# wenet-e2e/wesep

Hardware: AMD Instinct MI355X
Metric: utterances/sec (4 s, 16 kHz, 2-spk) fwd+bwd, pBSRNN (higher is better)
Workload: dtype bf16x3+fp16x2+fp16x1 split products (+fp8 lo terms), fp32 accumulate; 1 GPU; pBSRNN FiLM multi-fuse, 6 repeats, feature_dim 128, fixed 256-d embeddings; fwd + SI-SDR + bwd + per-tensor clip + Adam-L2; bf16x3 (x-projections, projections, d(hcat), BN / mask GEMMs) + fp16x2 (recurrent products of all four recurrence kernels, d(xn)) + fp16x1 (LSTM weight gradients); 2-byte saved gates / d(gates); fp32 accumulate; BPTT kernels: W_hh as fp16 hi + block-scaled FP8 lo; the lo term; rows_per_gpu=32, global_rows=32, samples_per_row=64000, parallelism=dp1

## Files before the change

### include/wesep_hip.h

```cpp
#ifndef WESEP_HIP_H_
#define WESEP_HIP_H_

#ifdef __cplusplus
extern "C" {
#endif

#define WS_ABI_VERSION 20
#define WS_OK 0
#define WS_ERR_INVALID (-1)
#define WS_ERR_LAUNCH (-2)

int ws_abi_version(void);
const char* ws_last_error(void);

#define WS_PROF_LSTM_FWD 0
#define WS_PROF_LSTM_BWD 1
#define WS_PROF_GEMM_NT 2
#define WS_PROF_GEMM_TN 3
#define WS_PROF_NKINDS 4
int ws_prof_enable(int on);
int ws_prof_collect(int kind, double* total_ms, long long* launches);
int ws_debug_dirty_lds(float value, int nblocks, int spins, float* sink, void* stream);
int ws_debug_occupy(int nblocks, int usec, const unsigned* stop, float* sink, void* stream);

// ... 592 lines not shown

#define WS_RESAMPLE_MAX_UD 1024
#define WS_RESAMPLE_MAX_K 4096
int ws_resample_geom(int rate_in, int rate_out, int* U, int* D, int* w, int* K);
int ws_resample_taps(int rate_in, int rate_out, float* taps);
int ws_resample_fwd(const float* x, long long ldx, int R, int n_in, int rate_in, int rate_out, const float* taps, float* y,
                    long long ldy, void* stream);
int ws_resample_stream_fwd(const float* buf, long long ldb, int R, int rate_in, int rate_out, const float* taps, int lead,
                           int n_valid, int final, int g_first, int n_out, float* y, long long ldy, int hist_from, int hist_len,
                           float* hist, long long ldh, void* stream);

typedef struct ws_resample_row {
  long long in_off, taps_off, out_off, hist_off;
  int U, D, K;
  int lead, n_valid, final, g_first, n_out, hist_from, hist_len;
} ws_resample_row;
typedef struct ws_rows_copy_row {
  long long src_off, dst_off;
  int len, fill;
} ws_rows_copy_row;
typedef struct ws_window_resample_row {
  long long in_off, taps_off, out_off;
  int U, D, K;
  int lead, n_valid, final, g_first, p_first, L, fill;
} ws_window_resample_row;
int ws_resample_stream_rows_fwd(const ws_resample_row* rows, const ws_resample_row* d_rows, int A, const float* buf,
                                long long n_buf, const float* taps, long long n_taps, float* y, long long n_y, float* hist,
                                long long n_hist, void* stream);
int ws_rows_copy_fwd(const ws_rows_copy_row* rows, const ws_rows_copy_row* d_rows, int A, const float* src, long long n_src,
                     float* dst, long long n_dst, void* stream);
int ws_window_resample_rows_fwd(const ws_window_resample_row* rows, const ws_window_resample_row* d_rows, int A, const float* buf,
                                long long n_buf, const float* taps, long long n_taps, float* y, long long n_y, void* stream);

#ifdef __cplusplus
}
#endif
#endif
```

### wesep_amd/_lib.py

```python
import ctypes as C
import os

import numpy as np
import torch

_HERE = os.path.dirname(os.path.abspath(__file__))
LIB_PATH = os.environ.get("WESEP_HIP_LIB") or os.path.join(_HERE, "libwesep_hip.so")

WS_OK = 0
PROF_LSTM_FWD, PROF_LSTM_BWD, PROF_GEMM_NT, PROF_GEMM_TN = 0, 1, 2, 3
LSTM_H = 256
ABI_VERSION = 20
GATES_F32, GATES_H2, GATES_H2S, GATES_H2F = 0, 1, 2, 3
DGATES_EXP = 8


def dgates_scale(amax_bits: int) -> float:
    e = (int(amax_bits) >> 23) & 0xFF
    return 1.0 if e in (0, 255) else 2.0 ** (min(max(DGATES_EXP + 254 - e, 1), 253) - 127)


LSTM_F32_MT1, LSTM_F32_MT2, LSTM_BF16X3, LSTM_BF16X3_BLK, LSTM_BF16X3_BLK16 = 1, 2, 3, 4, 5
LSTM_FWD_H2P = 16
LSTM_C16 = 32
# ... 53 lines not shown
    _fields_ = [(n, _p) for n in ("G", "X", "slab", "bslab")] + \
               [(n, _ll) for n in ("ldg", "slab_stride", "bslab_stride")] + \
               [(n, _i) for n in ("M", "Nn", "nsplit", "tiles_per_split")] + [("conv", ConvView)]


class GroupsGeom(C.Structure):
    _fields_ = [("band_w", _p), ("band_off", _p), ("gs1", _ll), ("gs2", _ll), ("rs", _ll),
                ("ngroups", _i), ("gdiv", _i), ("L", _i), ("W", _i), ("nbands", _i), ("pad_", _i)]


class LstmArgs(C.Structure):
    _fields_ = [(n, _p) for n in ("gates", "cbuf", "hcat", "dhcat", "wpack")] + \
               [(n, _ll) for n in ("sq_s1", "sq_s2", "step_rows")] + \
               [(n, _i) for n in ("nseq", "sq_div", "L", "mode")] + [("run_if", _p)] + \
               [("gates_in", _p), ("dgates", _p), ("gfmt", _i), ("rfmt", _i), ("amax", _p)] + \
               [("dxn", _p), ("dxn_dir_stride", _ll), ("wxpack", _p)]


class SeqMapC(C.Structure):
    _fields_ = [("sq_s1", _ll), ("sq_s2", _ll), ("step_rows", _ll), ("nseq", _i), ("sq_div", _i), ("L", _i), ("nvalid", _i)]


class GemmP2BArgs(C.Structure):
    _fields_ = [(n, _p) for n in ("A", "Wpack", "bias", "C", "A_bl", "stats", "gamma", "beta")] + \
               [("sm", SeqMapC)] + [(n, _ll) for n in ("lda", "st_m1", "st_m2", "st_base")] + \
               [(n, _i) for n in ("st_div1", "st_div2", "N", "K")] + [("run_if", _p), ("amax", _p), ("A_bl16", _p)]


class GemmB2PArgs(C.Structure):
    _fields_ = [(n, _p) for n in ("A", "Wpack", "bias", "R", "C")] + [("sm", SeqMapC), ("ldc", _ll), ("N", _i), ("K", _i),
                                                                         ("a_fmt", _i), ("pad_", _i), ("amax", _p), ("a16_out", _p)]


class FilmDesc(C.Structure):
    _fields_ = [("a", _p), ("b", _p), ("a0", _f), ("rows_per_r", _i)]


class GemmTNBArgs(C.Structure):
    _fields_ = [(n, _p) for n in ("G", "A0", "A1", "slab", "bslab", "aslab")] + \
               [(n, _ll) for n in ("slab_stride", "bslab_stride", "aslab_stride")] + \
               [(n, _i) for n in ("g_width", "g_off", "g_cols", "a0_width", "a0_off", "a0_cols", "a0_shift",
                                  "a1_width", "a1_off", "a1_cols", "a1_shift", "nblk", "L", "nsplit",
                                  "blocks_per_split", "g_fmt")] + [("amax", _p), ("a_fmt", _i), ("pad_", _i)]


class LstmClusterArgs(C.Structure):
    _fields_ = [(n, _p) for n in ("gates", "cbuf", "hcat", "dhcat", "whh_f", "whh_r", "xchg", "flags", "status")] + \
               [("nseq", _i), ("L", _i), ("dbg", _i), ("gfmt", _i), ("gates_in", _p)]


class LstmCluster2Args(C.Structure):
    _fields_ = [(n, _p) for n in ("gates", "cbuf", "hcat", "xn", "wcat", "bcat", "whh_f", "whh_r", "xchg", "tword", "status")] + \
               [("nseq", _i), ("L", _i), ("dbg", _i), ("rfmt", _i), ("dbg_buf", _p)]


class LstmPairArgs(C.Structure):
    _fields_ = [(n, _p) for n in ("gates", "cbuf", "dhcat", "wpack", "xchg", "flags", "status", "dbg_buf")] + \
               [("nseq", _i), ("L", _i), ("dbg", _i), ("gfmt", _i), ("dgates", _p), ("amax", _p), ("rfmt", _i), ("pad_", _i)]


class Bands(C.Structure):
    _fields_ = [("band_of_bin", _p), ("band_f0", _p), ("band_bw", _p), ("nband", _i), ("nbins", _i)]


GROUP_NT_DTYPE = np.dtype([("W", "<u8"), ("bias", "<u8"), ("gamma", "<u8"), ("beta", "<u8"),
                           ("a_off", "<i8"), ("c_off", "<i8"), ("st_base", "<i8"),
                           ("K", "<i4"), ("N", "<i4"), ("ldw", "<i4"), ("pad_", "<i4")])
GROUP_TN_DTYPE = np.dtype([("gamma", "<u8"), ("beta", "<u8"), ("g_off", "<i8"), ("a_off", "<i8"),
                           ("st_base", "<i8"), ("out_off", "<i8"), ("bout_off", "<i8"),
                           ("Nn", "<i4"), ("Kk", "<i4"), ("pad0_", "<i4"), ("pad1_", "<i4")])
TENSOR_REF_DTYPE = np.dtype([("param", "<u8"), ("grad", "<u8"), ("exp_avg", "<u8"),
                             ("exp_avg_sq", "<u8"), ("numel", "<i8")])
assert GROUP_NT_DTYPE.itemsize == 72 and GROUP_TN_DTYPE.itemsize == 72 and TENSOR_REF_DTYPE.itemsize == 40

class LstmFusedArgs(C.Structure):
    _fields_ = [("gates", _p), ("cbuf", _p), ("hcat", _p), ("xn", _p), ("wpack", _p), ("bias", _p),
                ("nseq", _i), ("L", _i), ("gfmt", _i), ("hfmt", _i)]


LSTM_FUSED_PACK_FLOATS = 2 * 8 * 24 * 4 * 2 * 64 * 4
LSTM_DX_PACK_FLOATS = 16 * (48 * 1024 + 64) // 4

_SIGS = {
    "ws_abi_version": (_i, []),
    "ws_last_error": (C.c_char_p, []),
    "ws_prof_enable": (_i, [_i]),
    "ws_prof_collect": (_i, [_i, C.POINTER(C.c_double), C.POINTER(_ll)]),
    "ws_debug_dirty_lds": (_i, [_f, _i, _i, _p, _p]),
    "ws_debug_occupy": (_i, [_i, _i, _p, _p, _p]),
    "ws_pack_w_f16": (_i, [_p, _i, _i, _ll, _i, _i, _p, _p]),
    "ws_pack_w_f16f8": (_i, [_p, _i, _i, _ll, _i, _p, _p]),
    "ws_gemm_nt": (_i, [C.POINTER(GemmNTArgs), _p]),
    "ws_gemm_tn": (_i, [C.POINTER(GemmTNArgs), _p]),
    "ws_reduce_slabs": (_i, [_p, _i, _ll, _ll, _p, _i, _ll, _p]),
    "ws_transpose": (_i, [_p, _i, _i, _ll, _p, _p]),
    "ws_group_stats": (_i, [_p, C.POINTER(GroupsGeom), _f, _p, _p]),
    "ws_group_stats_len": (_i, [_p, C.POINTER(GroupsGeom), _p, _i, _f, _p, _p]),
    "ws_gn_bwd_reduce": (_i, [_p, _p, _p, _p, _p, C.POINTER(GroupsGeom), _p, _p]),
    "ws_gn_bwd_apply": (_i, [_p, _p, _p, _p, _p, _p, _p, C.POINTER(GroupsGeom), _p, _p]),
    "ws_gn_param_grad": (_i, [_p, _p, _p, C.POINTER(GroupsGeom), _i, _p, _p]),
    "ws_gn_bwd_fused": (_i, [_p, _p, _p, _p, _p, C.POINTER(GroupsGeom), _i, _p, _p, _p, _p, _p]),
    "ws_gn_bwd_fused2": (_i, [_p, _p, _p, _p, _p, _p, C.POINTER(GroupsGeom), _i, _p, _p, _p, _p, _p]),
    "ws_gn_bwd_apply_pg": (_i, [_p, _p, _p, _p, _p, _p, C.POINTER(GroupsGeom), _p, _p, _p, _p, _p]),
    "ws_group_stats_film": (_i, [_p, C.POINTER(FilmDesc), C.POINTER(GroupsGeom), _f, _p, _p]),
    "ws_gn_bwd_reduce_film": (_i, [_p, C.POINTER(FilmDesc), _p, _p, _p, C.POINTER(GroupsGeom), _p, _p]),
    "ws_gn_bwd_apply_pg_film": (_i, [_p, C.POINTER(FilmDesc), _p, _p, _p, _p, _p, C.POINTER(GroupsGeom), _p, _p, _p, _p,
                                     _p, _p, _p, _p, _p]),
    "ws_lstm_pack": (_i, [_p, _p, _p, _p, _i, _p]),
    "ws_lstm_fwd": (_i, [C.POINTER(LstmArgs), _p]),
    "ws_lstm_bwd": (_i, [C.POINTER(LstmArgs), _p]),
    "ws_lstm_fwd_cluster": (_i, [C.POINTER(LstmClusterArgs), _p]),
    "ws_lstm_bwd_cluster": (_i, [C.POINTER(LstmClusterArgs), _p]),
    "ws_lstm_fwd_cluster2": (_i, [C.POINTER(LstmCluster2Args), _p]),
    "ws_lstm_pack_pair": (_i, [_p, _p, _p, _p]),
    "ws_lstm_pack_pair_f16": (_i, [_p, _p, _p, _p]),
    "ws_lstm_pack_pair_f8": (_i, [_p, _p, _p, _p]),
    "ws_lstm_pack_pair_f8mx": (_i, [_p, _p, _p, _p]),
    "ws_lstm_pack_bwd_f8": (_i, [_p, _p, _p, _p]),
    "ws_lstm_pack_dx_f8": (_i, [_p, _p, _p]),
    "ws_lstm_bwd_pair": (_i, [C.POINTER(LstmPairArgs), _p]),
    "ws_lstm_cat_ih": (_i, [_p, _p, _p, _p, _p, _p, _i, _p, _p, _p]),
    "ws_pack_w": (_i, [_p, _i, _i, _ll, _i, _i, _p, _p]),
    "ws_gemm_p2b": (_i, [C.POINTER(GemmP2BArgs), _p]),
    "ws_gemm_p2b_len": (_i, [C.POINTER(GemmP2BArgs), _p, _i, _p]),
    "ws_gemm_b2p": (_i, [C.POINTER(GemmB2PArgs), _p]),
    "ws_gemm_p2b_film": (_i, [C.POINTER(GemmP2BArgs), C.POINTER(FilmDesc), _p]),
    "ws_gemm_b2p_film": (_i, [C.POINTER(GemmB2PArgs), C.POINTER(FilmDesc), _p]),
    "ws_gemm_tnb": (_i, [C.POINTER(GemmTNBArgs), _p]),
    "ws_gemm_tnb_h16": (_i, [C.POINTER(GemmTNBArgs), _p]),
    "ws_stft_bandsplit": (_i, [_p, _i, _i, C.POINTER(Bands), _p, _p]),
    "ws_stft_bandsplit_len": (_i, [_p, _i, _i, _p, C.POINTER(Bands), _p, _p]),
    "ws_mask_istft_frames": (_i, [_p, _p, _i, _i, C.POINTER(Bands), _p, _p]),
    "ws_istft_ola": (_i, [_p, _i, _i, _i, _p, _p]),
    "ws_istft_ola_len": (_i, [_p, _i, _i, _i, _p, _p, _p]),
    "ws_mask_istft_bwd": (_i, [_p, _p, _p, _i, _i, _i, C.POINTER(Bands), _p, _p]),
    "ws_affine_fwd": (_i, [_p, _p, _p, _f, _ll, _i, _i, _p, _p]),
    "ws_affine_bwd": (_i, [_p, _p, _p, _f, _ll, _i, _i, _i, _p, _p, _p, _p, _p, _p, _p]),
    "ws_sisdr_fwd": (_i, [_p, _p, _i, _i, _f, _p, _p, _p]),
    "ws_sisdr_bwd": (_i, [_p, _p, _p, _p, _i, _i, _p, _p]),
    "ws_flat_stats": (_i, [_p, _i, _ll, C.c_float, _i, _p, _p, _p]),
    "ws_prelu_fwd": (_i, [_p, _p, _p, _ll, _i, _i, _p, _p]),
    "ws_prelu_bwd": (_i, [_p, _p, _p, _ll, _p, _p, _i, _p]),
    "ws_dwconv_fwd": (_i, [_p, _p, _p, _p, _p, _p, _i, _i, _i, _i, _i, _i, _p, _p]),
    "ws_dwconv_bwd": (_i, [_p, _p, _p, _p, _p, _p, _i, _i, _i, _i, _i, _i, _p, _i, _i, _p, _p]),
    "ws_dwconv_ex_fwd": (_i, [_p, _p, _p, _p, _p, _p, _i, _i, _i, _i, _i, _i, _i, _p, _p]),
    "ws_dwconv_ex_bwd": (_i, [_p, _p, _p, _p, _p, _p, _i, _i, _i, _i, _i, _i, _i, _p, _i, _i, _p, _p]),
    "ws_chan_sums": (_i, [_p, _p, _p, _i, _i, _i, _i, _i, _p, _p]),
    "ws_norm_ab": (_i, [_p, _p, _i, _i, _ll, _p, _p]),
    "ws_norm_bwd_apply_cl": (_i, [_p, _p, _p, _p, _p, _p, _ll, _i, _i, _p, _p]),
    "ws_maskmul_fwd": (_i, [_p, _ll, _p, _ll, _i, _p, _p]),
    "ws_maskmul_bwd": (_i, [_p, _p, _ll, _p, _ll, _i, _p, _ll, _p, _p]),
    "ws_relu_mask": (_i, [_p, _p, _ll, _p]),
    "ws_ola_fwd": (_i, [_p, _p, _i, _i, _i, _i, _i, _p, _p]),
    "ws_ola_bwd": (_i, [_p, _i, _i, _i, _i, _i, _p, _p]),
    "ws_sum_partial": (_i, [_p, _ll, _p, _i, _p]),
    "ws_bn_stats": (_i, [_p, _ll, _i, C.c_float, C.c_float, _p, _p, _i, _p, _p, _p]),
    "ws_bn_prelu_fwd": (_i, [_p, _p, _p, _p, _p, _p, _ll, _i, _p, _p, _p]),
    "ws_bn_bwd": (_i, [_p, _p, _p, _p, _ll, _i, _i, _p, _p, _p, _p]),
    "ws_maxpool3_fwd": (_i, [_p, _i, _i, _i, _p, _p]),
    "ws_maxpool3_bwd": (_i, [_p, _p, _i, _i, _i, _p, _p]),
# ... 155 lines not shown
```

### wesep_amd/dev.py

```python
import ctypes as C
import os
from typing import NamedTuple, Optional

import numpy as np
import torch

from . import _lib as L

BIG = 1 << 30


def gemm_mode() -> str:
    return os.environ.get("WESEP_GEMM", "bf16x3")


def _mode_bit(mode):
    return 4 if (mode or gemm_mode()) == "bf16x3" else 0
GN_EPS = float(np.finfo(np.float32).eps)


class Rows(NamedTuple):
    div: int
    s1: int
    s2: int
# ... 58 lines not shown
    ldp: int = 0


def _set_conv(a, conv: Optional[ConvView]):
    if conv is not None:
        a.conv.on = 1
        (a.conv.mode, a.conv.H, a.conv.W, a.conv.C, a.conv.Ho, a.conv.Wo, a.conv.k, a.conv.sh, a.conv.sw,
         a.conv.p, a.conv.dil, a.conv.ldp) = conv


def gemm_nt(*, A, a_rows: Rows, M: int, C_out, c_rows: Rows, N=0, K=0, W=None, ldw=0, bias=None,
            R=None, T=None, stats=None, gamma=None, beta=None, stat_map: Optional[StatMap] = None,
            act=0, groups=None, ngroups=0, max_n=0, vec=3, a_off=0, c_off=0, w_off=0, mode=None,
            conv: Optional[ConvView] = None):
    for n, t in (("A", A), ("W", W), ("bias", bias), ("C", C_out), ("R", R), ("T", T),
                 ("stats", stats), ("gamma", gamma), ("beta", beta)):
        _chk(t, n)
    a = L.GemmNTArgs()
    a.A, a.W, a.bias, a.C = _p(A, a_off), _p(W, w_off), _p(bias), _p(C_out, c_off)
    a.R, a.T = _p(R, c_off), _p(T, c_off)
    a.stats, a.gamma, a.beta = _p(stats), _p(gamma), _p(beta)
    a.groups = C.c_void_p(groups.data_ptr()) if groups is not None else None
    a.a_div, a.a_s1, a.a_s2 = a_rows
    a.c_div, a.c_s1, a.c_s2 = c_rows
    sm = stat_map or StatMap(1, 0, 1, 0, 0)
    a.st_div1, a.st_m1, a.st_div2, a.st_m2, a.st_base = sm
    a.M, a.N, a.K, a.ldw = M, N, K, ldw
    a.act, a.ngroups, a.max_n, a.vec = act, ngroups, max_n, vec | _mode_bit(mode)
    _set_conv(a, conv)
    if ALG is not None and groups is None:
        a_elems = (M // (conv.Ho * conv.Wo)) * conv.H * conv.W * conv.C if conv is not None else M * K
        _alg("gemm_nt", 4 * (a_elems + M * N * (1 + (R is not None) + (T is not None)) + N * K), 2 * M * N * K)
    L.check(L.lib().ws_gemm_nt(C.byref(a), L.stream_ptr()), "ws_gemm_nt")


def tn_splits(M: int):
    nsplit = max(1, min(64, M // 2048))
    rows = -(-M // nsplit)
    rows = -(-rows // 32) * 32
    nsplit = -(-M // rows)
    return nsplit, rows


def gemm_tn(*, G, g_rows: Rows, A, a_rows: Rows, M: int, slab, slab_stride: int, nsplit: int,
            rows_per_split: int, Nn=0, Kk=0, bslab=None, bslab_stride=0, out_off=0, bout_off=0,
            stats=None, gamma=None, beta=None, stat_map: Optional[StatMap] = None,
            shift_rows=0, seq_div=1, seq_len=1, groups=None, ngroups=0, max_n=0, max_k=0, vec=1,
            g_off=0, a_off=0, mode=None, conv: Optional[ConvView] = None):
    for n, t in (("G", G), ("A", A), ("slab", slab), ("bslab", bslab), ("stats", stats),
                 ("gamma", gamma), ("beta", beta)):
        _chk(t, n)
    a = L.GemmTNArgs()
    a.G, a.A, a.slab, a.bslab = _p(G, g_off), _p(A, a_off), _p(slab), _p(bslab)
    a.stats, a.gamma, a.beta = _p(stats), _p(gamma), _p(beta)
    a.groups = C.c_void_p(groups.data_ptr()) if groups is not None else None
    a.g_div, a.g_s1, a.g_s2 = g_rows
    a.a_div, a.a_s1, a.a_s2 = a_rows
    sm = stat_map or StatMap(1, 0, 1, 0, 0)
    a.st_div1, a.st_m1, a.st_div2, a.st_m2, a.st_base = sm
    a.slab_stride, a.bslab_stride, a.out_off, a.bout_off = slab_stride, bslab_stride, out_off, bout_off
    a.M, a.Nn, a.Kk, a.rows_per_split, a.nsplit = M, Nn, Kk, rows_per_split, nsplit
    a.shift_rows, a.seq_div, a.seq_len = shift_rows, seq_div, seq_len
    a.ngroups, a.max_n, a.max_k, a.vec = ngroups, max_n, max_k, vec | _mode_bit(mode)
    _set_conv(a, conv)
    if ALG is not None and groups is None:
        a_elems = (M // (conv.Ho * conv.Wo)) * conv.H * conv.W * conv.C if conv is not None else M * Kk
# ... 2045 lines not shown
```

### wesep_amd/functional.py

```python
import os

import numpy as np
import torch

from . import _lib as L
from . import dev
from .dev import BIG, Geom, Rows, SeqMap, StatMap, flat
from .blstm_core import (G4, H, PAIR_STAMPS, PackCache, WeightPacks, WGradBox, WGradCarrierFn, _NO_CACHE,
                         _PROBE_SAT, _cluster_dbg, _empty, _h2_probe, _pair_dbg, _pending, _probe_round, _reduce_new,
                         _side_stream, amax_word, band_dx, band_rfmt, blstm_bptt, blstm_dxn, blstm_forward,
                         blstm_weight_grads, consume_once, defer_wgrad, dxn_fmt, flush_deferred_wgrads, keep_for_side,
                         make_plan, mark_wgrads_ready, pair_rfmt, tnb_a16, weight_grads, wgrad_hold, zero_words)

NBIN = 257
HOP = 128


def _need_cuda(t, who):
    if not t.is_cuda:
        raise L.WesepHipError(f"{who}: wesep_amd has no CPU path; move the model and inputs to the GPU")


def _view_maps(view, R, K, Tf, N):
    if view == "time":
# ... 440 lines not shown

    @staticmethod
    def backward(ctx, dout):
        z, e, W = ctx.saved_tensors
        dout = dout.contiguous()
        R, K, Tf, N = z.shape
        E = e.shape[1]
        P = R * K * Tf
        d = z.device
        ns = _affine_splits(K * Tf)
        dc_slab = _empty(d, ns, R, N)
        dev.affine_bwd(dout, None, None, 1.0, P, K * Tf, N, ns, None, None, dc_slab)
        dc = _reduce_new(dc_slab, ns, R * N, (R, N))
        dW = _empty(d, N, N + E)
        nsplit, rps = dev.tn_splits(P)
        slab = _empty(d, nsplit, N * N)
        dev.gemm_tn(G=dout, g_rows=flat(N), A=z, a_rows=flat(N), M=P, Nn=N, Kk=N, slab=slab,
                    slab_stride=N * N, nsplit=nsplit, rows_per_split=rps)
        dev.reduce_slabs(slab, nsplit, N * N, N * N, dW, w=N, ldo=N + E)
        dWe, db = _lin_bwd_w(dc, e)
        dev.reduce_slabs(dWe, 1, N * E, N * E, dW, w=E, ldo=N + E, out_off=N)
        dz = _empty(d, R, K, Tf, N)
        WxT = _empty(d, N, N)
        dev.transpose(W, N, N, N + E, WxT)
        dev.gemm_nt(A=dout, a_rows=flat(N), M=P, N=N, K=N, W=WxT, ldw=N, C_out=dz, c_rows=flat(N))
        de = _lin_bwd_x(dc, W, src_off=N, rows=N, cols=E, lds=N + E) if ctx.needs_input_grad[1] else None
        return dz, de, dW, db


def mask_nn() -> bool:
    return dev.gemm_mode() == "bf16x3" and os.environ.get("WESEP_GEMM_NN", "1") != "0"


class BandPlan:

    def __init__(self, band_width, feature_dim, device):
        self.dev = device
        self.bands = dev.BandTables(band_width, device)
        self.bw = [int(b) for b in band_width]
        self.f0 = [int(f) for f in self.bands.f0_host]
        self.K = len(self.bw)
        self.N = feature_dim
        N = feature_dim
        H1 = 4 * N
        self.bn_woff = np.concatenate([[0], np.cumsum([N * 2 * b for b in self.bw])]).astype(np.int64)
        self.m_w3off = np.concatenate([[0], np.cumsum([4 * b * H1 for b in self.bw])]).astype(np.int64)
        self.m_b3off = np.concatenate([[0], np.cumsum([4 * b for b in self.bw])]).astype(np.int64)
        self.bn_wT = _empty(device, int(self.bn_woff[-1]))
        self.m_w1T = _empty(device, self.K * N * H1)
        self.m_w2T = _empty(device, self.K * H1 * H1)
        self.m_w3T = _empty(device, int(self.m_w3off[-1]))
        self._cache = {}

    def _up(self, arr):
        return L.upload_struct_array(arr, self.dev)

    def _key(self, params, R, Tf):
        return (R, Tf) + tuple(p.data_ptr() for p in params)

    def bn_desc(self, params, R, Tf):
        key = ("bn",) + self._key(params, R, Tf)
        if key not in self._cache:
            K, N = self.K, self.N
            nt = np.zeros(K, dtype=L.GROUP_NT_DTYPE)
            tn = np.zeros(K, dtype=L.GROUP_TN_DTYPE)
            dx = np.zeros(K, dtype=L.GROUP_NT_DTYPE)
            for g in range(K):
                gw, gb, cw, cb = params[4 * g:4 * g + 4]
                bw2 = 2 * self.bw[g]
                nt[g] = (cw.data_ptr(), cb.data_ptr(), gw.data_ptr(), gb.data_ptr(),
                         2 * self.f0[g], g * Tf * N, g, bw2, N, bw2, 0)
                tn[g] = (gw.data_ptr(), gb.data_ptr(), g * Tf * N, 2 * self.f0[g], g,
                         int(self.bn_woff[g]), g * N, N, bw2, 0, 0)
                dx[g] = (self.bn_wT.data_ptr() + 4 * int(self.bn_woff[g]), 0, 0, 0,
                         g * Tf * N, 2 * self.f0[g], 0, N, bw2, N, 0)
            self._cache = {k: v for k, v in self._cache.items() if k[0] != "bn"}
            self._cache[key] = (self._up(nt), self._up(tn), self._up(dx))
        return self._cache[key]

    def mask_desc(self, params, R, Tf):
        nn = mask_nn()
        key = ("mask", nn) + self._key(params, R, Tf)
        if key not in self._cache:
            K, N = self.K, self.N
            H1 = 4 * N
            M = R * Tf
            d = {n: np.zeros(K, dtype=L.GROUP_NT_DTYPE) for n in ("l1", "l2", "l3", "dh2", "dh1", "dxn")}
            t = {n: np.zeros(K, dtype=L.GROUP_TN_DTYPE) for n in ("w3", "w2", "w1")}
            gtab = np.zeros(K, dtype=np.uint64)
            for g in range(K):
                gw, gb, w1, b1, w2, b2, w3, b3 = params[8 * g:8 * g + 8]
                bw4 = 4 * self.bw[g]
                hoff = g * M * H1
                zoff = g * Tf * N
                gtab[g] = gw.data_ptr()
                d["l1"][g] = (w1.data_ptr(), b1.data_ptr(), gw.data_ptr(), gb.data_ptr(), zoff, hoff, g, N, H1, N, 0)
                d["l2"][g] = (w2.data_ptr(), b2.data_ptr(), 0, 0, hoff, hoff, 0, H1, H1, H1, 0)
                d["l3"][g] = (w3.data_ptr(), b3.data_ptr(), 0, 0, hoff, 4 * self.f0[g], 0, H1, bw4, H1, 0)
                if nn:
                    d["dh2"][g] = (w3.data_ptr(), 0, 0, 0, 4 * self.f0[g], hoff, 0, bw4, H1, H1, 0)
                    d["dh1"][g] = (w2.data_ptr(), 0, 0, 0, hoff, hoff, 0, H1, H1, H1, 0)
                    d["dxn"][g] = (w1.data_ptr(), 0, 0, 0, hoff, zoff, 0, H1, N, N, 0)
                else:
                    d["dh2"][g] = (self.m_w3T.data_ptr() + 4 * int(self.m_w3off[g]), 0, 0, 0,
                                   4 * self.f0[g], hoff, 0, bw4, H1, bw4, 0)
                    d["dh1"][g] = (self.m_w2T.data_ptr() + 4 * g * H1 * H1, 0, 0, 0, hoff, hoff, 0, H1, H1, H1, 0)
                    d["dxn"][g] = (self.m_w1T.data_ptr() + 4 * g * N * H1, 0, 0, 0, hoff, zoff, 0, H1, N, H1, 0)
                t["w3"][g] = (0, 0, 4 * self.f0[g], hoff, 0, int(self.m_w3off[g]), int(self.m_b3off[g]), bw4, H1, 0, 0)
                t["w2"][g] = (0, 0, hoff, hoff, 0, g * H1 * H1, g * H1, H1, H1, 0, 0)
                t["w1"][g] = (gw.data_ptr(), gb.data_ptr(), hoff, zoff, g, g * H1 * N, g * H1, H1, N, 0, 0)
            self._cache = {k: v for k, v in self._cache.items() if k[0] != "mask"}
            out = {k: self._up(v) for k, v in d.items()}
            out.update({"t" + k: self._up(v) for k, v in t.items()})
            out["gamma_tab"] = torch.from_numpy(gtab.view(np.int64)).to(self.dev)
            self._cache[key] = out
        return self._cache[key]


def _band_split_fwd(wav, plan, params, lengths=None, frames=None):
    R, T = wav.shape
    K, N = plan.K, plan.N
    Tf = 1 + T // HOP
    M = R * Tf
    d = wav.device
    xbs = _empty(d, M, 2 * NBIN)
    geo = Geom(R * K, K, Tf * 2 * NBIN, 0, 2 * NBIN, Tf, 128, K, plan.bands.bw2, plan.bands.off2)
    stats = _empty(d, R * K, 2)
    if lengths is None:
        dev.stft_bandsplit(wav, plan.bands, xbs)
        dev.group_stats(xbs, geo, stats)
    else:
        dev.stft_bandsplit(wav, plan.bands, xbs, lengths=lengths)
        dev.group_stats(xbs, geo, stats, glen=frames, glen_div=K)
    nt, _, _ = plan.bn_desc(params, R, Tf)
    z0 = _empty(d, R, K, Tf, N)
    dev.gemm_nt(A=xbs, a_rows=flat(2 * NBIN), M=M, C_out=z0, c_rows=Rows(Tf, K * Tf * N, N),
                stats=stats, stat_map=StatMap(Tf, K, 1, 0, 0), groups=nt, ngroups=K, max_n=N, vec=0)
    return z0, xbs, stats


def _mask_decode_fwd(z, xbs, plan, T, params, lengths=None, frames=None):
    R, K, Tf, N = z.shape
    H1 = 4 * N
    M = R * Tf
    d = z.device
    D = plan.mask_desc(params, R, Tf)
    geo = Geom(R * K, 1, Tf * N, 0, N, Tf, N, K)
    stats = _empty(d, R * K, 2)
    if lengths is None:
        dev.group_stats(z, geo, stats)
    else:
        dev.group_stats(z, geo, stats, glen=frames, glen_div=K)
    h1, h2 = _empty(d, K, M, H1), _empty(d, K, M, H1)
    dev.gemm_nt(A=z, a_rows=Rows(Tf, K * Tf * N, N), M=M, C_out=h1, c_rows=flat(H1), stats=stats,
                stat_map=StatMap(Tf, K, 1, 0, 0), act=1, groups=D["l1"], ngroups=K, max_n=H1)
    dev.gemm_nt(A=h1, a_rows=flat(H1), M=M, C_out=h2, c_rows=flat(H1), act=1, groups=D["l2"],
                ngroups=K, max_n=H1)
    m3 = _empty(d, M, 4 * NBIN)
    dev.gemm_nt(A=h2, a_rows=flat(H1), M=M, C_out=m3, c_rows=flat(4 * NBIN), groups=D["l3"],
                ngroups=K, max_n=4 * max(plan.bw))
    fr = _empty(d, M, 512)
    dev.mask_istft_frames(xbs, m3, R, Tf, plan.bands, fr)
    est = _empty(d, R, T)
    if lengths is None:
        dev.istft_ola(fr, R, Tf, T, est)
    else:
        dev.istft_ola(fr, R, Tf, T, est, lengths=lengths)
    return est, stats, h1, h2, m3


def band_split_ragged(wav, plan, params, lengths, frames):
    _need_cuda(wav, "BSRNN")
    return _band_split_fwd(wav.contiguous(), plan, [p.detach() for p in params], lengths, frames)[:2]


def mask_decode_ragged(z, xbs, plan, T, params, lengths, frames):
    _need_cuda(z, "BSRNN")
    return _mask_decode_fwd(z.contiguous(), xbs, plan, T, [p.detach() for p in params], lengths, frames)[0]


class BandSplitFn(torch.autograd.Function):

    @staticmethod
    def forward(ctx, wav, plan, *params):
        _need_cuda(wav, "BSRNN")
        wav = wav.contiguous()
        R, T = wav.shape
        Tf = 1 + T // HOP
        z0, xbs, stats = _band_split_fwd(wav, plan, params)
        ctx.save_for_backward(xbs, stats, *params)
# ... 17 lines not shown
        nsplit, rps = dev.tn_splits(M)
        wtot = int(plan.bn_woff[-1])
        slab, bslab = _empty(d, nsplit, wtot), _empty(d, nsplit, K * N)
        dev.gemm_tn(G=dz0, g_rows=Rows(Tf, K * Tf * N, N), A=xbs, a_rows=flat(2 * NBIN), M=M, slab=slab,
                    slab_stride=wtot, bslab=bslab, bslab_stride=K * N, nsplit=nsplit, rows_per_split=rps,
                    stats=stats, stat_map=smap, groups=tn, ngroups=K, max_n=N, max_k=128, vec=0)
        dW = _reduce_new(slab, nsplit, wtot, (wtot,))
        dB = _reduce_new(bslab, nsplit, K * N, (K * N,))
        for g in range(K):
            bw2 = 2 * plan.bw[g]
            dev.transpose(params[4 * g + 2].reshape(N, bw2), N, bw2, bw2, plan.bn_wT,
                          dst_off=int(plan.bn_woff[g]))
        dxn = _empty(d, M, 2 * NBIN)
        dev.gemm_nt(A=dz0, a_rows=Rows(Tf, K * Tf * N, N), M=M, C_out=dxn, c_rows=flat(2 * NBIN),
                    groups=dxd, ngroups=K, max_n=128, vec=3)
        ns2 = min(64, R)
        pslab = _empty(d, ns2, K, 2, 128)
        dev.gn_param_grad(xbs, dxn, stats, geo, ns2, pslab)
        dgb = _reduce_new(pslab, ns2, K * 2 * 128, (K, 2, 128))
        grads = []
        for g in range(K):
            bw2 = 2 * plan.bw[g]
            o = int(plan.bn_woff[g])
            grads += [dgb[g, 0, :bw2], dgb[g, 1, :bw2], dW[o:o + N * bw2].view(N, bw2, 1), dB[g * N:(g + 1) * N]]
        return (None, None) + tuple(grads)


class MaskDecodeFn(torch.autograd.Function):

    @staticmethod
    def forward(ctx, z, xbs, plan, T, *params):
        _need_cuda(z, "BSRNN")
        z = z.contiguous()
        est, stats, h1, h2, m3 = _mask_decode_fwd(z, xbs, plan, T, params)
        ctx.save_for_backward(z, xbs, stats, h1, h2, m3, *params)
        ctx.plan, ctx.T = plan, T
        return est

    @staticmethod
    def backward(ctx, dest):
        z, xbs, stats, h1, h2, m3 = ctx.saved_tensors[:6]
        params = ctx.saved_tensors[6:]
        plan, T = ctx.plan, ctx.T
        R, K, Tf, N = z.shape
        H1 = 4 * N
        M = R * Tf
        d = z.device
        D = plan.mask_desc(params, R, Tf)
        dest = dest.contiguous()
        dm3 = _empty(d, M, 4 * NBIN)
        dev.mask_istft_bwd(dest, xbs, m3, R, Tf, T, plan.bands, dm3)
        nsplit, rps = dev.tn_splits(M)
        maxb4 = 4 * max(plan.bw)
        w3tot, b3tot = int(plan.m_w3off[-1]), int(plan.m_b3off[-1])
        slab, bslab = _empty(d, nsplit, w3tot), _empty(d, nsplit, b3tot)
        dev.gemm_tn(G=dm3, g_rows=flat(4 * NBIN), A=h2, a_rows=flat(H1), M=M, slab=slab, slab_stride=w3tot,
                    bslab=bslab, bslab_stride=b3tot, nsplit=nsplit, rows_per_split=rps, groups=D["tw3"],
                    ngroups=K, max_n=maxb4, max_k=H1)
        dW3 = _reduce_new(slab, nsplit, w3tot, (w3tot,))
        dB3 = _reduce_new(bslab, nsplit, b3tot, (b3tot,))
        nn = mask_nn()
        vnn = 3 | (8 if nn else 0)
        if not nn:
            for g in range(K):
                bw4 = 4 * plan.bw[g]
                dev.transpose(params[8 * g + 6].reshape(bw4, H1), bw4, H1, H1, plan.m_w3T,
                              dst_off=int(plan.m_w3off[g]))
                dev.transpose(params[8 * g + 4].reshape(H1, H1), H1, H1, H1, plan.m_w2T, dst_off=g * H1 * H1)
                dev.transpose(params[8 * g + 2].reshape(H1, N), H1, N, N, plan.m_w1T, dst_off=g * N * H1)
        dh2 = _empty(d, K, M, H1)
        dev.gemm_nt(A=dm3, a_rows=flat(4 * NBIN), M=M, C_out=dh2, c_rows=flat(H1), T=h2, groups=D["dh2"],
                    ngroups=K, max_n=H1, vec=vnn)
        slab, bslab = _empty(d, nsplit, K * H1 * H1), _empty(d, nsplit, K * H1)
        dev.gemm_tn(G=dh2, g_rows=flat(H1), A=h1, a_rows=flat(H1), M=M, slab=slab, slab_stride=K * H1 * H1,
                    bslab=bslab, bslab_stride=K * H1, nsplit=nsplit, rows_per_split=rps, groups=D["tw2"],
                    ngroups=K, max_n=H1, max_k=H1)
        dW2 = _reduce_new(slab, nsplit, K * H1 * H1, (K, H1, H1, 1))
        dB2 = _reduce_new(bslab, nsplit, K * H1, (K, H1))
        dh1 = _empty(d, K, M, H1)
        dev.gemm_nt(A=dh2, a_rows=flat(H1), M=M, C_out=dh1, c_rows=flat(H1), T=h1, groups=D["dh1"],
                    ngroups=K, max_n=H1, vec=vnn)
        del dh2
        slab, bslab = _empty(d, nsplit, K * H1 * N), _empty(d, nsplit, K * H1)
        dev.gemm_tn(G=dh1, g_rows=flat(H1), A=z, a_rows=Rows(Tf, K * Tf * N, N), M=M, slab=slab,
                    slab_stride=K * H1 * N, bslab=bslab, bslab_stride=K * H1, nsplit=nsplit,
                    rows_per_split=rps, stats=stats, stat_map=StatMap(Tf, K, 1, 0, 0), groups=D["tw1"],
                    ngroups=K, max_n=H1, max_k=N)
        dW1 = _reduce_new(slab, nsplit, K * H1 * N, (K, H1, N, 1))
        dB1 = _reduce_new(bslab, nsplit, K * H1, (K, H1))
        del slab, bslab
        dxn = _empty(d, R, K, Tf, N)
        dev.gemm_nt(A=dh1, a_rows=flat(H1), M=M, C_out=dxn, c_rows=Rows(Tf, K * Tf * N, N), groups=D["dxn"],
                    ngroups=K, max_n=N, vec=vnn)
        del dh1
        geo = Geom(R * K, 1, Tf * N, 0, N, Tf, N, K)
        ab = _empty(d, R * K, 2)
        dev.gn_bwd_reduce(z, dxn, stats, geo, ab, gamma_tab=D["gamma_tab"])
        ns2 = min(64, R)
        pslab = _empty(d, ns2, K, 2, N)
        dev.gn_param_grad(z, dxn, stats, geo, ns2, pslab)
        dgb = _reduce_new(pslab, ns2, K * 2 * N, (K, 2, N))
        dz = torch.empty_like(z)
        dev.gn_bwd_apply(z, dxn, stats, ab, geo, dz, gamma_tab=D["gamma_tab"])
        grads = []
        for g in range(K):
            bw4 = 4 * plan.bw[g]
            o3, ob3 = int(plan.m_w3off[g]), int(plan.m_b3off[g])
            grads += [dgb[g, 0], dgb[g, 1], dW1[g], dB1[g], dW2[g], dB2[g],
                      dW3[o3:o3 + bw4 * H1].view(bw4, H1, 1), dB3[ob3:ob3 + bw4]]
        return (dz, None, None, None) + tuple(grads)


class SISDRFn(torch.autograd.Function):
    @staticmethod
    def forward(ctx, est, tgt, eps):
        _need_cuda(est, "SISDRLoss")
        est, tgt = est.contiguous().float(), tgt.contiguous().float()
        R = est.shape[0]
        rowstat = _empty(est.device, R, 8)
        loss = _empty(est.device, 1)
        dev.sisdr_fwd(est, tgt, rowstat, loss, eps)
        ctx.save_for_backward(est, tgt, rowstat)
        return loss.view(())

    @staticmethod
    def backward(ctx, gout):
# ... 5 lines not shown
```

Before: 359.7 utterances/s.

## Add pre-packed bf16x3 MFMA row GEMM for mask decoder layers

Adds a new grouped GEMM kernel that multiplies rows by weights pre-split into bf16 hi and lo parts and laid out in MFMA tiles. Weights are staged into LDS through buffer-to-LDS loads with double buffering. The kernel fuses the group-norm affine step, bias, tanh and the tanh-derivative epilogue. It replaces the generic gemm_nt for the mask decoder's l1/l2 forward GEMMs and the dh1/dxn backward GEMMs. Weight packing is cached and redone only when the weight versions, the weight epoch or the stream change, which adds bookkeeping and buffer memory and depends on that invalidation being correct.

After: 361.9 utterances/s, median of 6. No clear change (+0.6%).

```diff
diff --git a/include/wesep_hip.h b/include/wesep_hip.h
--- a/include/wesep_hip.h
+++ b/include/wesep_hip.h
@@ -648,6 +648,33 @@
 int ws_window_resample_rows_fwd(const ws_window_resample_row* rows, const ws_window_resample_row* d_rows, int A, const float* buf,
                                 long long n_buf, const float* taps, long long n_taps, float* y, long long n_y, void* stream);
 
+typedef struct ws_pack_rows_desc {
+  const float* W;
+  void* out;
+  long long ldw;
+  int N, K, trans, pad_;
+} ws_pack_rows_desc;
+int ws_pack_rows_w(const ws_pack_rows_desc* tab, int n, int max_elems, void* stream);
+
+typedef struct ws_group_rows {
+  const void* Wpack;
+  const float* bias;
+  const float* gamma;
+  const float* beta;
+  long long a_off, c_off, st_base;
+} ws_group_rows;
+typedef struct ws_gemm_rows_args {
+  const float* A;
+  float* C;
+  const float* T;
+  const float* stats;
+  const ws_group_rows* groups;
+  long long a_s1, a_s2, c_s1, c_s2, st_m1, st_m2;
+  int a_div, c_div, st_div1, st_div2;
+  int M, N, K, act, ngroups, pad_;
+} ws_gemm_rows_args;
+int ws_gemm_rows(const ws_gemm_rows_args* a, void* stream);
+
 #ifdef __cplusplus
 }
 #endif
diff --git a/wesep_amd/_lib.py b/wesep_amd/_lib.py
--- a/wesep_amd/_lib.py
+++ b/wesep_amd/_lib.py
@@ -109,6 +109,12 @@
                                                                          ("a_fmt", _i), ("pad_", _i), ("amax", _p), ("a16_out", _p)]
 
 
+class GemmRowsArgs(C.Structure):
+    _fields_ = [(n, _p) for n in ("A", "C", "T", "stats", "groups")] + \
+               [(n, _ll) for n in ("a_s1", "a_s2", "c_s1", "c_s2", "st_m1", "st_m2")] + \
+               [(n, _i) for n in ("a_div", "c_div", "st_div1", "st_div2", "M", "N", "K", "act", "ngroups", "pad_")]
+
+
 class FilmDesc(C.Structure):
     _fields_ = [("a", _p), ("b", _p), ("a0", _f), ("rows_per_r", _i)]
 
@@ -146,8 +152,13 @@
 GROUP_TN_DTYPE = np.dtype([("gamma", "<u8"), ("beta", "<u8"), ("g_off", "<i8"), ("a_off", "<i8"),
                            ("st_base", "<i8"), ("out_off", "<i8"), ("bout_off", "<i8"),
                            ("Nn", "<i4"), ("Kk", "<i4"), ("pad0_", "<i4"), ("pad1_", "<i4")])
+GROUP_ROWS_DTYPE = np.dtype([("Wpack", "<u8"), ("bias", "<u8"), ("gamma", "<u8"), ("beta", "<u8"),
+                             ("a_off", "<i8"), ("c_off", "<i8"), ("st_base", "<i8")])
+PACK_ROWS_DTYPE = np.dtype([("W", "<u8"), ("out", "<u8"), ("ldw", "<i8"), ("N", "<i4"), ("K", "<i4"), ("trans", "<i4"),
+                            ("pad_", "<i4")])
 TENSOR_REF_DTYPE = np.dtype([("param", "<u8"), ("grad", "<u8"), ("exp_avg", "<u8"),
                              ("exp_avg_sq", "<u8"), ("numel", "<i8")])
+assert GROUP_ROWS_DTYPE.itemsize == 56 and PACK_ROWS_DTYPE.itemsize == 40
 assert GROUP_NT_DTYPE.itemsize == 72 and GROUP_TN_DTYPE.itemsize == 72 and TENSOR_REF_DTYPE.itemsize == 40
 
 class LstmFusedArgs(C.Structure):
@@ -203,6 +214,8 @@
     "ws_gemm_b2p": (_i, [C.POINTER(GemmB2PArgs), _p]),
     "ws_gemm_p2b_film": (_i, [C.POINTER(GemmP2BArgs), C.POINTER(FilmDesc), _p]),
     "ws_gemm_b2p_film": (_i, [C.POINTER(GemmB2PArgs), C.POINTER(FilmDesc), _p]),
+    "ws_gemm_rows": (_i, [C.POINTER(GemmRowsArgs), _p]),
+    "ws_pack_rows_w": (_i, [_p, _i, _i, _p]),
     "ws_gemm_tnb": (_i, [C.POINTER(GemmTNBArgs), _p]),
     "ws_gemm_tnb_h16": (_i, [C.POINTER(GemmTNBArgs), _p]),
     "ws_stft_bandsplit": (_i, [_p, _i, _i, C.POINTER(Bands), _p, _p]),
diff --git a/wesep_amd/csrc/gemm_rows.hip b/wesep_amd/csrc/gemm_rows.hip
--- /dev/null
+++ b/wesep_amd/csrc/gemm_rows.hip
@@ -0,0 +1,212 @@
+#include "common.h"
+
+typedef __bf16 bf16x8 __attribute__((ext_vector_type(8)));
+typedef unsigned int u32x4 __attribute__((ext_vector_type(4)));
+
+__device__ __forceinline__ f32x16 mfma32r(bf16x8 a, bf16x8 b, f32x16 c) {
+  return __builtin_amdgcn_mfma_f32_32x32x16_bf16(a, b, c, 0, 0, 0);
+}
+
+__global__ void pack_rows_w_kernel(const ws_pack_rows_desc* __restrict__ tab) {
+  const ws_pack_rows_desc d = tab[blockIdx.y];
+  const int idx = blockIdx.x * blockDim.x + threadIdx.x;
+  if (idx >= d.N * d.K / 8) return;
+  const int lane = idx & 63, r = idx >> 6;
+  const int nt = r & 3, ks = (r >> 2) & 3, s = r >> 4;
+  const int nst = d.K / 64, st = s % nst, cg = s / nst;
+  const int n = 128 * cg + 32 * nt + (lane & 31), k0 = 64 * st + 16 * ks + 8 * (lane >> 5);
+  bf16x8 hi, lo;
+#pragma unroll
+  for (int j = 0; j < 8; ++j) {
+    const float v = d.trans ? d.W[(long long)(k0 + j) * d.ldw + n] : d.W[(long long)n * d.ldw + k0 + j];
+    hi[j] = (__bf16)v;
+    lo[j] = (__bf16)(v - (float)hi[j]);
+  }
+  bf16x8* o = reinterpret_cast<bf16x8*>(d.out) + (long long)r * 128 + lane;
+  o[0] = hi;
+  o[64] = lo;
+}
+
+extern "C" int ws_pack_rows_w(const ws_pack_rows_desc* tab, int n, int max_elems, void* stream) {
+  WS_REQUIRE(tab && n > 0, "ws_pack_rows_w: table / n (n=%d)", n);
+  WS_REQUIRE(max_elems == 128 * 128 || max_elems == 128 * 512 || max_elems == 512 * 512,
+             "ws_pack_rows_w: max_elems = max N * K over the table, N and K in {128, 512} (got %d)", max_elems);
+  hipLaunchKernelGGL(pack_rows_w_kernel, dim3(max_elems / 8 / 256, n), dim3(256), 0, (hipStream_t)stream, tab);
+  return ws_check_launch("ws_pack_rows_w");
+}
+
+template <bool NORM, bool HAST>
+__global__ __launch_bounds__(512, 4) void gemm_rows_kernel(const ws_gemm_rows_args p) {
+  __shared__ __attribute__((aligned(16))) u32x4 wl[2][2048];
+  __shared__ long long cofl[8][32];
+  const int tid = threadIdx.x, lane = tid & 63, i = lane & 31, half = lane >> 5;
+  const int w = __builtin_amdgcn_readfirstlane(tid >> 6);
+  const int K = p.K, nstage = K / 64, ncg = p.N / 128;
+  const int nrb = (p.M + 255) / 256;
+  const int chunk = blockIdx.x / (8 * ncg), rem = blockIdx.x - chunk * (8 * ncg);
+  const int rbg = chunk * 8 + (rem & 7), cg = rem >> 3;
+  if (rbg >= nrb * p.ngroups) return;
+  const int gi = rbg / nrb, rb = rbg - gi * nrb;
+  const ws_group_rows g = p.groups[gi];
+  const int m = rb * 256 + w * 32 + i;
+  const bool valid = m < p.M;
+  const int mm = valid ? m : p.M - 1;
+  if (half == 0) cofl[w][i] = valid ? g.c_off + ws_row_off(mm, p.c_div, p.c_s1, p.c_s2) + cg * 128 : -1;
+  const float* arow = p.A + g.a_off + ws_row_off(mm, p.a_div, p.a_s1, p.a_s2) + 8 * half;
+  float mean = 0.f, rstd = 1.f;
+  if (NORM) {
+    const long long s = (long long)(mm / p.st_div1) * p.st_m1 + (long long)(mm % p.st_div2) * p.st_m2 + g.st_base;
+    mean = p.stats[2 * s];
+    rstd = p.stats[2 * s + 1];
+  }
+  const unsigned char* wbase = reinterpret_cast<const unsigned char*>(g.Wpack) + (long long)cg * nstage * 32768;
+  const __amdgpu_buffer_rsrc_t wsr =
+      __builtin_amdgcn_make_buffer_rsrc(const_cast<unsigned char*>(wbase), 0, (unsigned)nstage * 32768u, 0x00020000);
+  auto wstage = [&](int st, int buf) {
+#pragma unroll
+    for (int q = 0; q < 4; ++q)
+      __builtin_amdgcn_raw_ptr_buffer_load_lds(wsr, (__attribute__((address_space(3))) void*)&wl[buf][(w * 4 + q) * 64], 16, lane * 16,
+                                               (st * 2048 + (w * 4 + q) * 64) * 16, 0, 0);
+  };
+  f32x4 an[4];
+  auto load_a = [&](int st, int hs) {
+    const float* a2 = arow + st * 64 + hs * 32;
+#pragma unroll
+    for (int ks = 0; ks < 2; ++ks) {
+      an[2 * ks] = *reinterpret_cast<const f32x4*>(a2 + 16 * ks);
+      an[2 * ks + 1] = *reinterpret_cast<const f32x4*>(a2 + 16 * ks + 4);
+    }
+  };
+  wstage(0, 0);
+  load_a(0, 0);
+  asm volatile("s_waitcnt vmcnt(0)" ::: "memory");
+  __syncthreads();
+
+  f32x16 acc[4];
+#pragma unroll
+  for (int t = 0; t < 4; ++t)
+#pragma unroll
+    for (int r = 0; r < 16; ++r) acc[t][r] = 0.f;
+
+  for (int st = 0; st < nstage; ++st) {
+    const int cur = st & 1;
+#pragma unroll
+    for (int hs = 0; hs < 2; ++hs) {
+      f32x4 ac[4];
+#pragma unroll
+      for (int q = 0; q < 4; ++q) ac[q] = an[q];
+      if (hs == 0 && st + 1 < nstage) wstage(st + 1, cur ^ 1);
+      if (hs == 0) load_a(st, 1);
+      else if (st + 1 < nstage) load_a(st + 1, 0);
+#pragma unroll
+      for (int ksl = 0; ksl < 2; ++ksl) {
+        const int ks = hs * 2 + ksl;
+        f32x4 v0 = ac[2 * ksl], v1 = ac[2 * ksl + 1];
+        if (NORM) {
+          const int k0 = st * 64 + ks * 16 + 8 * half;
+          const f32x4 g0 = *reinterpret_cast<const f32x4*>(g.gamma + k0), g1 = *reinterpret_cast<const f32x4*>(g.gamma + k0 + 4);
+          const f32x4 b0 = *reinterpret_cast<const f32x4*>(g.beta + k0), b1 = *reinterpret_cast<const f32x4*>(g.beta + k0 + 4);
+          v0 = (v0 - mean) * rstd * g0 + b0;
+          v1 = (v1 - mean) * rstd * g1 + b1;
+        }
+        bf16x8 ah, al;
+#pragma unroll
+        for (int j = 0; j < 4; ++j) {
+          ah[j] = (__bf16)v0[j];
+          al[j] = (__bf16)(v0[j] - (float)ah[j]);
+          ah[4 + j] = (__bf16)v1[j];
+          al[4 + j] = (__bf16)(v1[j] - (float)ah[4 + j]);
+        }
+        const u32x4* wt = &wl[cur][ks * 512 + lane];
+#pragma unroll
+        for (int nt = 0; nt < 4; ++nt) {
+          const bf16x8 bh = __builtin_bit_cast(bf16x8, wt[(nt * 2) * 64]);
+          const bf16x8 bl = __builtin_bit_cast(bf16x8, wt[(nt * 2 + 1) * 64]);
+          acc[nt] = mfma32r(ah, bh, acc[nt]);
+          acc[nt] = mfma32r(ah, bl, acc[nt]);
+          acc[nt] = mfma32r(al, bh, acc[nt]);
+        }
+      }
+    }
+    asm volatile("s_waitcnt vmcnt(0)" ::: "memory");
+    __syncthreads();
+  }
+
+  float* stg = reinterpret_cast<float*>(&wl[0][0]) + w * 2048;
+  const float* T = p.T;
+#pragma unroll
+  for (int pass = 0; pass < 2; ++pass) {
+#pragma unroll
+    for (int t = 0; t < 2; ++t) {
+#pragma unroll
+      for (int r = 0; r < 16; ++r) {
+        const int mr = (r & 3) + 8 * (r >> 2) + 4 * half;
+        stg[mr * 64 + t * 32 + i] = acc[2 * pass + t][r];
+      }
+    }
+    __syncthreads();
+    const int c4 = lane & 15, r0 = lane >> 4;
+    const int n = cg * 128 + pass * 64 + 4 * c4;
+    f32x4 bv = {0.f, 0.f, 0.f, 0.f};
+    if (g.bias) bv = *reinterpret_cast<const f32x4*>(g.bias + n);
+#pragma unroll
+    for (int hk = 0; hk < 2; ++hk) {
+      f32x4 v[4], tv[4];
+      long long off[4];
+#pragma unroll
+      for (int k = 0; k < 4; ++k) {
+        const int mr = r0 + 4 * (4 * hk + k);
+        const long long co = cofl[w][mr];
+        off[k] = co >= 0 ? co + pass * 64 + 4 * c4 : -1;
+        v[k] = *reinterpret_cast<const f32x4*>(stg + mr * 64 + 4 * c4);
+        if (g.bias) {
+#pragma unroll
+          for (int j = 0; j < 4; ++j) v[k][j] += bv[j];
+        }
+        if (HAST && off[k] >= 0) tv[k] = *reinterpret_cast<const f32x4*>(T + off[k]);
+      }
+#pragma unroll
+      for (int k = 0; k < 4; ++k) {
+        if (off[k] < 0) continue;
+        f32x4 o = v[k];
+#pragma unroll
+        for (int j = 0; j < 4; ++j) {
+          if (p.act == 1) o[j] = tanhf(o[j]);
+          if (HAST) o[j] *= (1.f - tv[k][j] * tv[k][j]);
+        }
+        *reinterpret_cast<f32x4*>(p.C + off[k]) = o;
+      }
+    }
+    __syncthreads();
+  }
+}
+
+extern "C" int ws_gemm_rows(const ws_gemm_rows_args* a, void* stream) {
+  WS_REQUIRE(a && a->A && a->C && a->groups, "ws_gemm_rows: null pointer");
+  WS_REQUIRE(a->K == 128 || a->K == 512, "ws_gemm_rows: K must be 128 or 512 (got %d)", a->K);
+  WS_REQUIRE(a->N == 128 || a->N == 512, "ws_gemm_rows: N must be 128 or 512 (got %d)", a->N);
+  WS_REQUIRE(a->M > 0 && a->ngroups > 0 && a->ngroups <= 65535, "ws_gemm_rows: M > 0, 0 < ngroups <= 65535 (M=%d, ngroups=%d)", a->M,
+             a->ngroups);
+  WS_REQUIRE(a->act == 0 || a->act == 1, "ws_gemm_rows: act 0 (none) or 1 (tanh) (got %d)", a->act);
+  WS_REQUIRE(a->a_div > 0 && a->c_div > 0, "ws_gemm_rows: row maps (a_div=%d, c_div=%d)", a->a_div, a->c_div);
+  WS_REQUIRE((a->a_s1 & 3) == 0 && (a->a_s2 & 3) == 0 && (a->c_s1 & 3) == 0 && (a->c_s2 & 3) == 0 && ((size_t)a->A & 15) == 0 &&
+                 ((size_t)a->C & 15) == 0 && ((size_t)a->T & 15) == 0,
+             "ws_gemm_rows: 16-byte row pieces (strides %% 4 == 0, A / C / T aligned)");
+  WS_REQUIRE(!a->stats || (a->st_div1 > 0 && a->st_div2 > 0), "ws_gemm_rows: norm args (st_div1=%d, st_div2=%d)", a->st_div1, a->st_div2);
+  WS_REQUIRE((const void*)a->A != (const void*)a->C, "ws_gemm_rows: C must not alias A");
+  const long long nrb = (a->M + 255) / 256;
+  const long long nblk = ((nrb * a->ngroups + 7) / 8) * 8 * (a->N / 128);
+  WS_REQUIRE(nblk < (1ll << 31), "ws_gemm_rows: too many workgroups");
+  hipStream_t s = (hipStream_t)stream;
+  ws_prof_begin(WS_PROF_GEMM_NT, s);
+  if (a->stats && a->T)
+    hipLaunchKernelGGL((gemm_rows_kernel<true, true>), dim3((unsigned)nblk), dim3(512), 0, s, *a);
+  else if (a->stats)
+    hipLaunchKernelGGL((gemm_rows_kernel<true, false>), dim3((unsigned)nblk), dim3(512), 0, s, *a);
+  else if (a->T)
+    hipLaunchKernelGGL((gemm_rows_kernel<false, true>), dim3((unsigned)nblk), dim3(512), 0, s, *a);
+  else
+    hipLaunchKernelGGL((gemm_rows_kernel<false, false>), dim3((unsigned)nblk), dim3(512), 0, s, *a);
+  ws_prof_end(WS_PROF_GEMM_NT, s);
+  return ws_check_launch("ws_gemm_rows");
+}
diff --git a/wesep_amd/dev.py b/wesep_amd/dev.py
--- a/wesep_amd/dev.py
+++ b/wesep_amd/dev.py
@@ -114,6 +114,25 @@
         a_elems = (M // (conv.Ho * conv.Wo)) * conv.H * conv.W * conv.C if conv is not None else M * K
         _alg("gemm_nt", 4 * (a_elems + M * N * (1 + (R is not None) + (T is not None)) + N * K), 2 * M * N * K)
     L.check(L.lib().ws_gemm_nt(C.byref(a), L.stream_ptr()), "ws_gemm_nt")
+
+
+def gemm_rows(*, A, a_rows: Rows, M: int, C_out, c_rows: Rows, N: int, K: int, groups, ngroups: int, T=None, stats=None,
+              stat_map: Optional[StatMap] = None, act=0):
+    for n, t in (("A", A), ("C", C_out), ("T", T), ("stats", stats)):
+        _chk(t, n)
+    a = L.GemmRowsArgs()
+    a.A, a.C, a.T, a.stats = _p(A), _p(C_out), _p(T), _p(stats)
+    a.groups = C.c_void_p(groups.data_ptr())
+    a.a_div, a.a_s1, a.a_s2 = a_rows
+    a.c_div, a.c_s1, a.c_s2 = c_rows
+    sm = stat_map or StatMap(1, 0, 1, 0, 0)
+    a.st_div1, a.st_m1, a.st_div2, a.st_m2 = sm[:4]
+    a.M, a.N, a.K, a.act, a.ngroups = M, N, K, act, ngroups
+    L.check(L.lib().ws_gemm_rows(C.byref(a), L.stream_ptr()), "ws_gemm_rows")
+
+
+def pack_rows_w(table, n: int, max_elems: int):
+    L.check(L.lib().ws_pack_rows_w(C.c_void_p(table.data_ptr()), n, max_elems, L.stream_ptr()), "ws_pack_rows_w")
 
 
 def tn_splits(M: int):
diff --git a/wesep_amd/functional.py b/wesep_amd/functional.py
--- a/wesep_amd/functional.py
+++ b/wesep_amd/functional.py
@@ -496,6 +496,11 @@
     return dev.gemm_mode() == "bf16x3" and os.environ.get("WESEP_GEMM_NN", "1") != "0"
 
 
+def mask_rows(device) -> bool:
+    return (dev.gemm_mode() == "bf16x3" and torch.device(device).type == "cuda"
+            and os.environ.get("WESEP_MASK_ROWS", "1") != "0")
+
+
 class BandPlan:
 
     def __init__(self, band_width, feature_dim, device):
@@ -515,6 +520,7 @@
         self.m_w2T = _empty(device, self.K * H1 * H1)
         self.m_w3T = _empty(device, int(self.m_w3off[-1]))
         self._cache = {}
+        self.m_packs, self._pack_tab, self._pack_key, self._pack_sig, self._pack_bwd = None, None, None, None, False
 
     def _up(self, arr):
         return L.upload_struct_array(arr, self.dev)
@@ -542,9 +548,37 @@
             self._cache[key] = (self._up(nt), self._up(tn), self._up(dx))
         return self._cache[key]
 
+    def _mask_pack_bufs(self):
+        if self.m_packs is None:
+            N, H1 = self.N, 4 * self.N
+            self.m_packs = {"l1": _empty(self.dev, self.K * H1 * N), "l2": _empty(self.dev, self.K * H1 * H1),
+                            "dh1": _empty(self.dev, self.K * H1 * H1), "dxn": _empty(self.dev, self.K * N * H1)}
+        return self.m_packs
+
+    def mask_packs(self, params, bwd):
+        K, N = self.K, self.N
+        H1 = 4 * N
+        ws = [params[8 * g + o] for g in range(K) for o in (2, 4)]
+        ptrs = tuple(w.data_ptr() for w in ws)
+        bufs = self._mask_pack_bufs()
+        if ptrs != self._pack_key:
+            tab = np.zeros(4 * K, dtype=L.PACK_ROWS_DTYPE)
+            for g in range(K):
+                w1, w2 = ptrs[2 * g], ptrs[2 * g + 1]
+                tab[g] = (w1, bufs["l1"].data_ptr() + 4 * g * H1 * N, N, H1, N, 0, 0)
+                tab[K + g] = (w2, bufs["l2"].data_ptr() + 4 * g * H1 * H1, H1, H1, H1, 0, 0)
+                tab[2 * K + g] = (w2, bufs["dh1"].data_ptr() + 4 * g * H1 * H1, H1, H1, H1, 1, 0)
+                tab[3 * K + g] = (w1, bufs["dxn"].data_ptr() + 4 * g * N * H1, N, N, H1, 1, 0)
+            self._pack_tab, self._pack_key, self._pack_sig = self._up(tab), ptrs, None
+        sig = (dev.weight_epoch(), torch.cuda.current_stream().cuda_stream) + tuple(w._version for w in ws)
+        if sig != self._pack_sig or (bwd and not self._pack_bwd):
+            dev.pack_rows_w(self._pack_tab, 4 * K if bwd else 2 * K, H1 * H1)
+            self._pack_sig, self._pack_bwd = sig, bool(bwd)
+
     def mask_desc(self, params, R, Tf):
         nn = mask_nn()
-        key = ("mask", nn) + self._key(params, R, Tf)
+        rows = mask_rows(self.dev)
+        key = ("mask", nn, rows) + self._key(params, R, Tf)
         if key not in self._cache:
             K, N = self.K, self.N
             H1 = 4 * N
@@ -575,6 +609,14 @@
                 t["w1"][g] = (gw.data_ptr(), gb.data_ptr(), hoff, zoff, g, g * H1 * N, g * H1, H1, N, 0, 0)
             self._cache = {k: v for k, v in self._cache.items() if k[0] != "mask"}
             out = {k: self._up(v) for k, v in d.items()}
+            if rows:
+                bufs = self._mask_pack_bufs()
+                for n, wsz in (("l1", H1 * N), ("l2", H1 * H1), ("dh1", H1 * H1), ("dxn", N * H1)):
+                    r = np.zeros(K, dtype=L.GROUP_ROWS_DTYPE)
+                    for g in range(K):
+                        r[g] = (bufs[n].data_ptr() + 4 * g * wsz,) + tuple(int(d[n][g][f]) for f in
+                                                                         ("bias", "gamma", "beta", "a_off", "c_off", "st_base"))
+                    out["r" + n] = self._up(r)
             out.update({"t" + k: self._up(v) for k, v in t.items()})
             out["gamma_tab"] = torch.from_numpy(gtab.view(np.int64)).to(self.dev)
             self._cache[key] = out
@@ -603,7 +645,7 @@
     return z0, xbs, stats
 
 
-def _mask_decode_fwd(z, xbs, plan, T, params, lengths=None, frames=None):
+def _mask_decode_fwd(z, xbs, plan, T, params, lengths=None, frames=None, bwd=False):
     R, K, Tf, N = z.shape
     H1 = 4 * N
     M = R * Tf
@@ -616,10 +658,16 @@
     else:
         dev.group_stats(z, geo, stats, glen=frames, glen_div=K)
     h1, h2 = _empty(d, K, M, H1), _empty(d, K, M, H1)
-    dev.gemm_nt(A=z, a_rows=Rows(Tf, K * Tf * N, N), M=M, C_out=h1, c_rows=flat(H1), stats=stats,
-                stat_map=StatMap(Tf, K, 1, 0, 0), act=1, groups=D["l1"], ngroups=K, max_n=H1)
-    dev.gemm_nt(A=h1, a_rows=flat(H1), M=M, C_out=h2, c_rows=flat(H1), act=1, groups=D["l2"],
-                ngroups=K, max_n=H1)
+    if mask_rows(d):
+        plan.mask_packs(params, bwd)
+        dev.gemm_rows(A=z, a_rows=Rows(Tf, K * Tf * N, N), M=M, C_out=h1, c_rows=flat(H1), N=H1, K=N, stats=stats,
+                      stat_map=StatMap(Tf, K, 1, 0, 0), act=1, groups=D["rl1"], ngroups=K)
+        dev.gemm_rows(A=h1, a_rows=flat(H1), M=M, C_out=h2, c_rows=flat(H1), N=H1, K=H1, act=1, groups=D["rl2"], ngroups=K)
+    else:
+        dev.gemm_nt(A=z, a_rows=Rows(Tf, K * Tf * N, N), M=M, C_out=h1, c_rows=flat(H1), stats=stats,
+                    stat_map=StatMap(Tf, K, 1, 0, 0), act=1, groups=D["l1"], ngroups=K, max_n=H1)
+        dev.gemm_nt(A=h1, a_rows=flat(H1), M=M, C_out=h2, c_rows=flat(H1), act=1, groups=D["l2"],
+                    ngroups=K, max_n=H1)
     m3 = _empty(d, M, 4 * NBIN)
     dev.gemm_nt(A=h2, a_rows=flat(H1), M=M, C_out=m3, c_rows=flat(4 * NBIN), groups=D["l3"],
                 ngroups=K, max_n=4 * max(plan.bw))
@@ -703,7 +751,7 @@
     def forward(ctx, z, xbs, plan, T, *params):
         _need_cuda(z, "BSRNN")
         z = z.contiguous()
-        est, stats, h1, h2, m3 = _mask_decode_fwd(z, xbs, plan, T, params)
+        est, stats, h1, h2, m3 = _mask_decode_fwd(z, xbs, plan, T, params, bwd=any(ctx.needs_input_grad))
         ctx.save_for_backward(z, xbs, stats, h1, h2, m3, *params)
         ctx.plan, ctx.T = plan, T
         return est
@@ -749,8 +797,13 @@
         dW2 = _reduce_new(slab, nsplit, K * H1 * H1, (K, H1, H1, 1))
         dB2 = _reduce_new(bslab, nsplit, K * H1, (K, H1))
         dh1 = _empty(d, K, M, H1)
-        dev.gemm_nt(A=dh2, a_rows=flat(H1), M=M, C_out=dh1, c_rows=flat(H1), T=h1, groups=D["dh1"],
-                    ngroups=K, max_n=H1, vec=vnn)
+        rows = mask_rows(d)
+        if rows:
+            plan.mask_packs(params, True)
+            dev.gemm_rows(A=dh2, a_rows=flat(H1), M=M, C_out=dh1, c_rows=flat(H1), N=H1, K=H1, T=h1, groups=D["rdh1"], ngroups=K)
+        else:
+            dev.gemm_nt(A=dh2, a_rows=flat(H1), M=M, C_out=dh1, c_rows=flat(H1), T=h1, groups=D["dh1"],
+                        ngroups=K, max_n=H1, vec=vnn)
         del dh2
         slab, bslab = _empty(d, nsplit, K * H1 * N), _empty(d, nsplit, K * H1)
         dev.gemm_tn(G=dh1, g_rows=flat(H1), A=z, a_rows=Rows(Tf, K * Tf * N, N), M=M, slab=slab,
@@ -761,8 +814,12 @@
         dB1 = _reduce_new(bslab, nsplit, K * H1, (K, H1))
         del slab, bslab
         dxn = _empty(d, R, K, Tf, N)
-        dev.gemm_nt(A=dh1, a_rows=flat(H1), M=M, C_out=dxn, c_rows=Rows(Tf, K * Tf * N, N), groups=D["dxn"],
-                    ngroups=K, max_n=N, vec=vnn)
+        if rows:
+            dev.gemm_rows(A=dh1, a_rows=flat(H1), M=M, C_out=dxn, c_rows=Rows(Tf, K * Tf * N, N), N=N, K=H1, groups=D["rdxn"],
+                          ngroups=K)
+        else:
+            dev.gemm_nt(A=dh1, a_rows=flat(H1), M=M, C_out=dxn, c_rows=Rows(Tf, K * Tf * N, N), groups=D["dxn"],
+                        ngroups=K, max_n=N, vec=vnn)
         del dh1
         geo = Geom(R * K, 1, Tf * N, 0, N, Tf, N, K)
         ab = _empty(d, R * K, 2)
```
